# una-auxme/MeshGraphNets.jl

Measured on AMD Instinct MI355X. Metric: processor-step edges/s, higher is better.
Workload: dtype f32; 1 GPU; M-1M jittered-grid triangulation 1000x1000: N=1000000 nodes, E=5992002 directed edges, L=128, hidden_layers=2, 15 processor steps per bench step, fp32 storage, fp16x2 split MFMA (every fp32 operand = two fp16 pieces after a power-of-two scaling per weight chunk / per activation row, three exact piece products per fp32 product on v_mfma_f32_32x32x16_f16), fp32 accumulate; held to the fp32 tolerance; partition=single partition, edge_order=engine re-sorts by receiver once per trajectory (mgn_set_graph)

## Files before the change

### meshgraphnets.jl_amd/csrc/kernels.h

```cpp
#pragma once
#include <hip/hip_runtime.h>
#include <stdint.h>

namespace mgn {

constexpr int TILE = 32;
constexpr int MAX_CHUNKS = 9;

enum { T_B1 = 0, T_B2, T_B3, T_GAMMA, T_BETA, T_BQ, T_LN, T_COUNT };

struct GenMlp {
    const float* chunk[4];
    const float* tabs;
    int32_t nmid;
    int32_t use;
};

struct EdgeArgs {
    const int32_t* snd;
    const int32_t* rcv;
    int64_t E;
    int32_t ntiles;
    const float* P;
    const float* Q;
// ... 46 lines not shown
    float h2_s[9], h2_rs[9], h2_b2pos;
};

struct EncNodeArgs {
    int32_t n, ntiles;
    const int32_t* gid;
    const float* srcA; int32_t wa;
    const float* srcB; int32_t wb;
    const float* scale;
    const float* shift;
    const float* w1f;
    float* V; float* P; float* Q;
    const float* chunk[MAX_CHUNKS];
    const float* tabs;
    GenMlp gen;
    const uint16_t* splith[4];
    float h2_rs[4];
};

struct EncEdgeArgs {
    int64_t E; int32_t ntiles;
    const int64_t* gid;
    const float* ef; int32_t Fe;
    const float* scale; const float* shift;
    const float* w1f;
    float* Elat;
    const float* chunk[MAX_CHUNKS];
    const float* tabs;
    GenMlp gen;
    const uint16_t* splith[2];
    float h2_rs[2];
};

struct DecArgs {
    int32_t n, ntiles;
    const float* V;
    const float* w3f;
    const float* b3;
    int32_t O;
    const float* oscale; const float* oshift;
    const float* mask;
    const int32_t* gid;
    float* out;
    const float* chunk[MAX_CHUNKS];
    const float* tabs;
    GenMlp gen;
    const uint16_t* splith[2];
    float h2_rs[2];
};

struct BfEdgeArgs {
    const int32_t* snd; const int32_t* rcv; int64_t E; int32_t ntiles; int32_t tile0;
    const uint16_t* P; const uint16_t* Q;
    uint16_t* Elat; uint16_t* AGG;
    uint16_t* CARRY;
    const uint16_t* chunk[3];
    const float* tabs;
    unsigned long long* stamps;
};
struct BfNodeArgs {
    int32_t n, ntiles; const int32_t* rowptr;
    uint16_t* V; const uint16_t* AGG; const uint16_t* CARRY; uint16_t* P; uint16_t* Q;
    const uint16_t* chunk[7];
    const float* tabs;
    int64_t zero_row; int32_t tile0;
    const int32_t* rowptr2; const uint16_t* AGG2; const uint16_t* CARRY2; int64_t zero_row2;
};
hipError_t launch_edge_bf16(const BfEdgeArgs& a, hipStream_t s);
hipError_t launch_node_bf16(const BfNodeArgs& a, hipStream_t s);
hipError_t launch_project_bf16(const BfNodeArgs& a, hipStream_t s);
hipError_t launch_tile_f32_to_bf16(const float* src, uint16_t* dst, int64_t ntiles, hipStream_t s);
hipError_t launch_tile_bf16_to_f32(const uint16_t* src, float* dst, int64_t ntiles, hipStream_t s);
hipError_t launch_scatter_prows(const float* src, int src_stride , float* dst, int64_t row0, int64_t rows, int L, hipStream_t s);
hipError_t launch_scatter_prows16(const uint16_t* src, int src_stride , uint16_t* dst, int64_t row0, int64_t rows, hipStream_t s);
bool prows_blocked();
hipError_t launch_gather_rows16(const uint16_t* src, const int32_t* idx, uint16_t* dst, int64_t rows, int dst_stride , hipStream_t s);

struct LaunchCfg { int blocks; int threads; size_t lds; };
hipError_t launch_node_split_h(const NodeArgs& a, const LaunchCfg& lc, hipStream_t s);
hipError_t launch_project_split_h(const NodeArgs& a, const LaunchCfg& lc, hipStream_t s);
hipError_t launch_edge_ring_h(const EdgeArgs& a, const LaunchCfg& lc, hipStream_t s);
size_t edge_ring_h_lds();
int edge_ring_h_streamed();
hipError_t launch_edge_ring(const EdgeArgs& a, const LaunchCfg& lc, hipStream_t s);
hipError_t launch_node_split(const NodeArgs& a, const LaunchCfg& lc, hipStream_t s);
hipError_t launch_project_split(const NodeArgs& a, const LaunchCfg& lc, hipStream_t s);

struct LinComb {
    int n;
    float c[7];
    const float* k[7];
};
hipError_t launch_lincomb(float* out, const float* u, const LinComb& lc, float dt, int64_t n, hipStream_t s);
hipError_t launch_overwrite(float* x, const float* frame, const uint8_t* mask, int64_t N, int O, hipStream_t s);
int errnorm_partials();
hipError_t launch_errnorm(const float* u, const float* unew, const LinComb& lc, float dt, float atol, float rtol, int64_t n,
                          double* partial, hipStream_t s);

bool launch_is_small(int ntiles);
bool node_split_size(int ntiles);
bool launch_is_small_edge(int ntiles_e);
int coop16_enabled();
int set_c16_edge_tiles(int t);
bool ring_hs_default();
bool coop16_size(int ntiles_e, int ntiles_n, bool ring_hs = false);
int last_edge_kernel();
int last_node_kernel();
int set_fp32_split(int on);
int fp32_split_enabled();
int set_split_f16(int on);
int split_f16_enabled();
int set_c16_split(int on);
int c16_split_enabled();
int set_c16_row_tiles(int rt);
int set_kernel_path(int p);
int get_kernel_path();
hipError_t launch_edge_step(int L, const EdgeArgs& a, hipStream_t s);
hipError_t launch_node_step(int L, const NodeArgs& a, hipStream_t s);
hipError_t launch_project(int L, const NodeArgs& a, hipStream_t s);
hipError_t launch_node_project_fused(int L, const NodeArgs& a, hipStream_t s, bool* launched);
hipError_t launch_node_ring_hs(const NodeArgs& a, const LaunchCfg& lc, hipStream_t s);
int node_ring_hs_enabled();
hipError_t launch_enc_node(int L, const EncNodeArgs& a, hipStream_t s);
hipError_t launch_enc_edge(int L, const EncEdgeArgs& a, hipStream_t s);
hipError_t launch_decode(int L, const DecArgs& a, hipStream_t s);
hipError_t launch_gather_rows(const float* src, const int32_t* idx, float* dst, int64_t rows, int L, int dst_stride , hipStream_t s);
hipError_t launch_rows_to_tiles(const float* src, const int64_t* gid64, const int32_t* gid32, float* dst, int64_t rows, int L, hipStream_t s);
hipError_t launch_tiles_to_rows(const float* src, const int64_t* gid64, const int32_t* gid32, float* dst, int64_t rows, int L, hipStream_t s);
hipError_t launch_randn_rows(float* dst, const int64_t* gid64, const int32_t* gid32, int64_t rows, int L,
                             uint64_t seed, hipStream_t s);
int kernels_prow_block();
int split_prow_block();
int checksum_partials();
hipError_t launch_checksum(const float* src, int64_t n, double* partials, hipStream_t s);

}
```

### meshgraphnets.jl_amd/csrc/kernels.hip

```cpp
#include "frag.hpp"
#include "kernels.h"
#include "tile_common.hpp"
#include "split_common.hpp"

#include <cstdlib>
#include <mutex>
#include <unordered_map>

namespace mgn {


template <int NT>
DEVINL void gen_hidden(f32x16 (&acc)[NT], f32x16 (&y)[NT], const GenMlp& g, int lane, int h) {
    constexpr int L = 32 * NT;
    relu_frag<NT>(acc);
    for (int m = 0; m < g.nmid; ++m) {
        tab_frag<NT>(y, g.tabs + m * L, h);
        mfma_chunk<NT, false>(y, acc, g.chunk[m], lane);
        relu_frag<NT>(y);
#pragma unroll
        for (int t = 0; t < NT; ++t) acc[t] = y[t];
    }
}
template <int NT>
// ... 2513 lines not shown

static int g_last_edge_kernel = 0;
int last_edge_kernel() { return g_last_edge_kernel; }
#define SET_LAST_EDGE(A, CODE)                                                            \
    do {                                                                                  \
        if (2 * (int64_t)(A).ntiles * TILE >= (A).E) g_last_edge_kernel = (CODE);         \
    } while (0)

hipError_t launch_edge_step(int L, const EdgeArgs& a, hipStream_t s) {
    if (a.ntiles <= 0) return hipSuccess;
    if (a.gen.use && a.ElatSrc) return hipErrorInvalidValue;
    if (a.gen.use) SET_LAST_EDGE(a, 1);
    if (a.gen.use) DISPATCH_GEN(L, (k_edge_step<4, 0, true>), (k_edge_step<2, 0, true>), (k_edge_step<1, 0, true>), a, a.ntiles);
    const int nres = resident_chunks(L, 3);
    LaunchCfg lc = tile_launch(L, a.ntiles, nres);
    if (a.c16 && L == 128 && a.chunk_t[0]) {
        SET_LAST_EDGE(a, 2);
        const int nht = 2 * a.ntiles;
        int rt = g_c16_rt ? g_c16_rt : (nht + num_cus() - 1) / num_cus();
        const bool sp16 = g_fp32_split && (g_c16_split & 1) && a.split16[0];
        const int rt_max = (sp16 && !a.bf && !g_c16_rt) ? 6 : 3;
        rt = rt < 1 ? 1 : (rt > rt_max ? rt_max : rt);
        LaunchCfg c16{(nht + rt - 1) / rt, 256, (size_t)rt * 2 * 8 * 64 * 16 + (size_t)rt * 2 * 64 * 4};
        if (g_fp32_split && (g_c16_split & 1) && a.split16[0] && (rt >= 2 || (g_c16_split & 4))) {
            c16.lds = (size_t)rt * 2 * 12 * 64 * 16 + (size_t)rt * 2 * 64 * 4;
            const bool h2 = g_split_f16 && a.split16h[0] && rt <= 4;
            SET_LAST_EDGE(a, h2 ? 15 : 12);
#define C16E(RT_, BF_) (h2 ? launch_k(k_edge_coop16m<RT_, BF_, 2>, a, c16, s) : launch_k(k_edge_coop16m<RT_, BF_, 1>, a, c16, s))
            if (a.bf) {
                if (rt == 3) return C16E(3, true);
                if (rt == 2) return C16E(2, true);
                return C16E(1, true);
            }
            if (rt == 6) return C16E(6, false);
            if (rt == 5) return C16E(5, false);
            if (rt == 4) return C16E(4, false);
            if (rt == 3) return C16E(3, false);
            if (rt == 2) return C16E(2, false);
            return C16E(1, false);
#undef C16E
        }
        if (a.bf) {
            if (rt == 3) return launch_k(k_edge_coop16m<3, true>, a, c16, s);
            if (rt == 2) return launch_k(k_edge_coop16m<2, true>, a, c16, s);
            return launch_k(k_edge_coop16m<1, true>, a, c16, s);
        }
        if (rt == 3) return launch_k(k_edge_coop16m<3, false>, a, c16, s);
        if (rt == 2) return launch_k(k_edge_coop16m<2, false>, a, c16, s);
        return launch_k(k_edge_coop16m<1, false>, a, c16, s);
    }
    if (a.ElatSrc) return hipErrorInvalidValue;
    static const int coop_edge_ring_env = [] { const char* e = getenv("MGN_COOP_EDGE_TILES_PER_CU_RING"); return e ? atoi(e) : 0; }();
    const bool ring_ok = L == 128 && g_fp32_split == 1 && a.split[0] && g_path == 0;
    const int coop_edge_ring = coop_edge_ring_env > 0 ? coop_edge_ring_env : ((ring_ok && g_split_f16 && a.splith[0] && edge_ring_h_streamed()) ? 2 : 3);
    if (coop_ok(L, a.ntiles, a.chunk_t, true) && !(ring_ok && a.ntiles > coop_edge_ring * num_cus())) {
        SET_LAST_EDGE(a, 3);
        LaunchCfg c4{a.ntiles, 256, coop_lds()};
        return coop_fence(a.ntiles) ? launch_k(k_edge_coop<true>, a, c4, s) : launch_k(k_edge_coop<false>, a, c4, s);
    }
    if (L == 128) {
        if (small_launch(a.ntiles) && !(ring_ok && a.ntiles > coop_edge_ring * num_cus())) {
            SET_LAST_EDGE(a, 4);
            lc.lds = (size_t)T_COUNT * L * 4 + 64;
            return launch_k(k_edge_step<4, 0>, a, lc, s);
        }
        if (g_fp32_split && a.split[0] && g_path == 0) {
            LaunchCfg ls = lc;
            ls.lds = (size_t)3 * 32768 + (size_t)3 * 16384 + (size_t)T_COUNT * L * 4 + 64;
            static const int ring_waves = [] { const char* e = getenv("MGN_RING_WAVES"); return e ? atoi(e) : 0; }();
            bool four = a.ntiles <= 20 * num_cus();
            if (g_split_f16 && a.splith[0] && edge_ring_h_streamed()) {
                const int r4 = (a.ntiles + 4 * num_cus() - 1) / (4 * num_cus()), r8 = (a.ntiles + 8 * num_cus() - 1) / (8 * num_cus());
                four = 0.62 * r4 < (double)r8;
            }
            if (ring_waves == 4 || (ring_waves == 0 && four)) {
                ls.threads = 256;
                const int rounds = (a.ntiles + 4 * num_cus() - 1) / (4 * num_cus());
                int blocks = (a.ntiles + 4 * rounds - 1) / (4 * rounds);
                if (blocks > num_cus()) blocks = num_cus();
                ls.blocks = ((blocks + NUM_XCD - 1) / NUM_XCD) * NUM_XCD;
            }
            if (g_split_f16 && a.splith[0]) {
                ls.lds = edge_ring_h_lds();
                SET_LAST_EDGE(a, edge_ring_h_streamed() ? (ls.threads == 256 ? 17 : 16) : (ls.threads == 256 ? 14 : 13));
                return launch_edge_ring_h(a, ls, s);
            }
            SET_LAST_EDGE(a, ls.threads == 256 ? 8 : 7);
            return launch_edge_ring(a, ls, s);
        }
        SET_LAST_EDGE(a, 9);
        lc.lds += (size_t)MGN_EDGE_JR * 64 * 4 * 4;
        const int nw = lc.blocks * (lc.threads / 64);
        const int rem = a.ntiles % nw, rounds = a.ntiles / nw;
        if (g_tail_coop && g_path == 0 && a.chunk_t[0] && rounds >= MGN_SPREAD_ROUNDS && rem > 0 && rem * 10 < nw * 6) {
            EdgeArgs body = a, tail = a;
            body.ntiles = a.ntiles - rem;
            tail.tile0 = a.tile0 + body.ntiles;
            tail.ntiles = rem;
            const hipError_t e = launch_k(k_edge_step<4, 2>, body, lc, s);
            if (e != hipSuccess) return e;
            LaunchCfg c4{rem, 256, coop_lds()};
            return launch_k(k_edge_coop<false>, tail, c4, s);
        }
        return launch_k(k_edge_step<4, 2>, a, lc, s);
    }
    if (L == 64) return launch_k(k_edge_step<2, 3>, a, lc, s);
    if (L == 32) return launch_k(k_edge_step<1, 3>, a, lc, s);
    return hipErrorInvalidValue;
}
static int g_last_node_kernel = 0;
int last_node_kernel() { return g_last_node_kernel; }
hipError_t launch_node_step(int L, const NodeArgs& a, hipStream_t s) {
    if (a.ntiles <= 0) return hipSuccess;
    if (a.mode != 2) g_last_node_kernel = a.gen.use ? 1 : (a.c16 && L == 128 && a.chunk_t[0]) ? 2 : coop_ok(L, a.ntiles, a.chunk_t) ? 3 : 7;
    if (a.gen.use) {
        if (a.mode == 2) return launch_project(L, a, s);
        if (a.AGG2) {
            if (a.mode == 1) return hipErrorInvalidValue;
            DISPATCH_GEN(L, (k_node_step<4, 0, false, 2, true>), (k_node_step<2, 0, false, 2, true>), (k_node_step<1, 0, false, 2, true>), a, a.ntiles);
        }
        if (a.mode == 1) DISPATCH_GEN(L, (k_node_step<4, 0, true, 1, true>), (k_node_step<2, 0, true, 1, true>), (k_node_step<1, 0, true, 1, true>), a, a.ntiles);
        DISPATCH_GEN(L, (k_node_step<4, 0, false, 1, true>), (k_node_step<2, 0, false, 1, true>), (k_node_step<1, 0, false, 1, true>), a, a.ntiles);
    }
    if (a.c16 && L == 128 && a.chunk_t[0]) {
        LaunchCfg c16{2 * a.ntiles, 256, (size_t)4 * 8 * 64 * 16 + 2 * 64 * 4};
        if (g_fp32_split && (g_c16_split & 2) && a.split16[0] && (!a.AGG2 || a.split16[6])) {
            c16.lds = (size_t)4 * 12 * 64 * 16 + 2 * 64 * 4;
            if (a.mode != 2) g_last_node_kernel = 8;
            if (g_split_f16 && a.split16h[0] && (!a.AGG2 || a.split16h[6])) {
                if (a.bf) return a.AGG2 ? launch_k(k_node_coop16<2, true, 2>, a, c16, s) : launch_k(k_node_coop16<1, true, 2>, a, c16, s);
                return a.AGG2 ? launch_k(k_node_coop16<2, false, 2>, a, c16, s) : launch_k(k_node_coop16<1, false, 2>, a, c16, s);
            }
            if (a.bf) return a.AGG2 ? launch_k(k_node_coop16<2, true, 1>, a, c16, s) : launch_k(k_node_coop16<1, true, 1>, a, c16, s);
            return a.AGG2 ? launch_k(k_node_coop16<2, false, 1>, a, c16, s) : launch_k(k_node_coop16<1, false, 1>, a, c16, s);
        }
        if (a.bf) return a.AGG2 ? launch_k(k_node_coop16<2, true>, a, c16, s) : launch_k(k_node_coop16<1, true>, a, c16, s);
        return a.AGG2 ? launch_k(k_node_coop16<2, false>, a, c16, s) : launch_k(k_node_coop16<1, false>, a, c16, s);
    }
    const bool split_node = L == 128 && a.mode == 0 && a.split[0] && (!a.AGG2 || a.split[6]) && node_split_size(a.ntiles);
    if (g_node16_mid && g_fp32_split && (g_c16_split & 2) && g_path == 0 && L == 128 && !a.bf && !a.AGG2 && a.mode != 2 && a.split16[0] &&
        coop_ok(L, a.ntiles, a.chunk_t) && !split_node) {
        LaunchCfg c16{2 * a.ntiles, 256, (size_t)4 * 12 * 64 * 16 + 2 * 64 * 4};
        g_last_node_kernel = 9;
        if (g_split_f16 && a.split16h[0]) return launch_k(k_node_coop16<1, false, 2, 5>, a, c16, s);
        return launch_k(k_node_coop16<1, false, 1, 5>, a, c16, s);
    }
    if (coop_ok(L, a.ntiles, a.chunk_t) && !split_node) {
        LaunchCfg c4{a.ntiles, 256, coop_lds()};
        if (coop_fence(a.ntiles)) return a.AGG2 ? launch_k(k_node_coop<true, true>, a, c4, s) : launch_k(k_node_coop<false, true>, a, c4, s);
        return a.AGG2 ? launch_k(k_node_coop<true, false>, a, c4, s) : launch_k(k_node_coop<false, false>, a, c4, s);
    }
    if (a.mode == 2) return launch_project(L, a, s);
    const bool proj = a.mode == 1;
    if (split_node) {
        LaunchCfg ls = tile_launch(L, a.ntiles, 2);
        ls.lds = (size_t)4 * 16384 * 2 + (size_t)T_COUNT * L * 4 + 64;
        if (g_split_f16 && a.splith[0] && !a.AGG2) {
            g_last_node_kernel = 10;
            return launch_node_split_h(a, ls, s);
        }
        g_last_node_kernel = a.AGG2 ? 6 : 5;
        return launch_node_split(a, ls, s);
    }
    const int nres = resident_chunks(L, proj ? 6 : 4);
    const LaunchCfg lc = tile_launch(L, a.ntiles, nres);
    if (a.AGG2) {
        if (proj) return hipErrorInvalidValue;
// ... 196 lines not shown
```

### meshgraphnets.jl_amd/csrc/split.hip

```cpp
#include <cstdlib>

#include "kernels.h"
#include "tile_common.hpp"
#include "split_common.hpp"

namespace mgn {

#ifndef MGN_SP_CARRY
#define MGN_SP_CARRY 1
#endif
#ifndef MGN_SP_BUFFER
#define MGN_SP_BUFFER 1
#endif

template <int D> struct SpRing { u32x4 r2[D], r3[D]; };
template <bool G2, bool G3, bool RELU, int D, bool G1 = false, int OFF = 0, bool PRIMED = false, bool NEXT = false>
DEVINL void sp_layer_otf(f32x16 (&acc)[4], const f32x16 (&in)[4], const u32x4* p1, const u32x4* p2, const u32x4* p3, int lane,
                         SpRing<D>* carry = nullptr, const u32x4* nx2 = nullptr, const u32x4* nx3 = nullptr) {
    const u32x4* w1 = p1 + lane;
    const u32x4* w2 = p2 + lane;
    const u32x4* w3 = p3 + lane;
#if MGN_SP_BUFFER
    const N16Buf b1 = n16_buf(G1 ? p1 : nullptr), b2 = n16_buf(G2 ? p2 : nullptr), b3 = n16_buf(G3 ? p3 : nullptr);
    const unsigned voff = (unsigned)lane * 16u;
// ... 1061 lines not shown
        asm volatile("s_nop 1");
        RG_SCAN_LEVEL(acc, c1, "row_shr:1 row_mask:0xf bank_mask:0xf");
        RG_SCAN_LEVEL(acc, c2s, "row_shr:2 row_mask:0xf bank_mask:0xf");
        RG_SCAN_LEVEL(acc, c4, "row_shr:4 row_mask:0xf bank_mask:0xf");
#if MGN_RINGH_SCAN_SKIP
        if (__builtin_amdgcn_ballot_w64(c8) != 0)
#endif
        {
            RG_SCAN_LEVEL(acc, c8, "row_shr:8 row_mask:0xf bank_mask:0xf");
        }
        RG_SCAN_LEVEL(acc, cx, "row_bcast:15 row_mask:0xa bank_mask:0xf");
        PHASE_FENCE();
        EST(5);
        const bool tail = valid && ((c == 31) || (reff != rnext));
        const int r_first = __builtin_amdgcn_readfirstlane(reff);
        const bool sl = (start == 0) && (ix.r_before == r_first);
        const bool sr = (c == 31) && (ix.r_after == reff);
        const bool to_carry = sl || sr;
        f32x4* dst = to_carry ? prow_ptr(a.CARRY, (int64_t)2 * tile + (sl ? 0 : 1), L, h) : tile_ptr(a.AGG, r >> 5, L, 32 * h + (r & 31));
#if defined(MGN_WHATIF_H) && (MGN_WHATIF_H & 32)
        if (tail && a.E < 0) store_frag<NT>(dst, to_carry ? STRIDE_PROW : STRIDE_TILE, acc);
#else
        if (tail) store_frag_pol<NT, MGN_AGG_STORE>(dst, to_carry ? STRIDE_PROW : STRIDE_TILE, acc);
#endif
        EST(6);
        PHASE_FENCE();
#if defined(MGN_WHATIF_H) && (MGN_WHATIF_H & 64)
        zero_frag<NT>(acc);
#elif defined(MGN_WHATIF_H) && (MGN_WHATIF_H & 8)
        load_frag<NT>(acc, prow_ptr(a.Q, lane & 31, L, h), STRIDE_PROW);
#else
        load_frag<NT>(acc, prow_ptr(a.Q, ixn.r >= 0 ? ixn.r : 0, L, h), STRIDE_PROW);
#endif
#if MGN_RINGH_ESTORE_LAST
        PHASE_FENCE();
#if defined(MGN_WHATIF_H) && (MGN_WHATIF_H & 2)
        if (valid && a.E < 0) ring_store_e(etile, er);
#else
        if (valid) ring_store_e(etile, er);
#endif
#endif
        EST(7);
        ix = ixn;
        tw.tile += tw.stride;
    }
}

constexpr int HS_W = 4;
#ifndef MGN_HS_PREMUL
#define MGN_HS_PREMUL 0
#endif
#ifndef MGN_HS_REQ_STEP
#define MGN_HS_REQ_STEP 0
#endif
#ifndef MGN_HS_AHEAD
#define MGN_HS_AHEAD 4
#endif
template <int NCH>
struct RsT {
    static constexpr int W = HS_W;
    static constexpr int WPL = 32 / W;
    static constexpr int NW = NCH * WPL;
    static constexpr int NB = 3;
    static constexpr int BUF = 2 * W * 64;
    static constexpr int AHEAD = MGN_HS_AHEAD;
    static constexpr int SLOTS = AHEAD - 1;
    static_assert(NW % NB == 0 && NW % SLOTS == 0 && AHEAD >= 3, "static window -> buffer / slot mapping");
};
typedef RsT<3> Rs;
template <int LYR>
DEVINL RhFrag rs_first(const u32x4* ring) {
    constexpr int b = (Rs::WPL * LYR) % Rs::NB;
    RhFrag f;
    f.h = ring[b * Rs::BUF];
    f.l = ring[b * Rs::BUF + 64];
    return f;
}
template <int NCH>
struct RsSrcT {
    const u32x4* w[NCH];
};
typedef RsSrcT<3> RsSrc;
DEVINL const u32x4* rs_src(const u32x4* chunk, int w, int e) { return chunk + ((e >> 6) & 1) * 2048 + (w * Rs::W + (e >> 7)) * 64 + (e & 63); }
template <int LYR, int FIN, int RFS = 0, int NWV = 8, bool WRAP = false, int NCH = 3, bool PREMUL = false>
DEVINL void hs_layer_ring(f32x16 (&acc)[4], f32x16 (&in)[4], u32x4* ring, const RsSrcT<NCH>& src, RhFrag& nx, u32x4 (&pend)[Rs::SLOTS][Rs::BUF / (NWV * 64)], int lane,
                          int tid, float sx, float cfin = 0.f, const float* btab = nullptr, const f32x4* rf = nullptr, const N16Buf* rfb = nullptr, int rfs_rt = 0, float premul = 1.f) {
    constexpr int ROT = 2;
    constexpr int W = Rs::W, WPL = Rs::WPL, NW = RsT<NCH>::NW, BUF = Rs::BUF, NB = Rs::NB;
    constexpr int LPT = BUF / (NWV * 64);
    f32x4 side[2 * ROT];
    if constexpr (!WRAP && RFS > 0) {
#pragma unroll
        for (int m = 0; m < 2 * ROT; ++m) side[m] = rf[m * RFS];
    }
    auto bias = [&](int sn, int u) {
        f32x2 b = {0.f, 0.f};
        if constexpr (FIN == 2) b = *reinterpret_cast<const f32x2*>(btab + 8 * (4 * (sn >> 1) + 2 * (sn & 1) + (u >> 1)) + 2 * (u & 1));
        return b;
    };
    unsigned ph[4], pl[4];
#pragma unroll
    for (int u = 0; u < 4; ++u) {
        const f32x2 b = bias(0, u);
        h2_split_pair<FIN>(ph[u], pl[u], in[0][2 * u], in[0][2 * u + 1], sx, cfin, b[0], b[1]);
    }
    unsigned voff[LPT];
#pragma unroll
    for (int i = 0; i < LPT; ++i) {
        const int e = i * NWV * 64 + tid;
        voff[i] = (unsigned)((((e >> 6) & 1) * 2048 + (e >> 7) * 64 + (e & 63)) * 16);
        asm volatile("" : "+v"(voff[i]));
    }
    __builtin_amdgcn_sched_barrier(0);
#pragma unroll
    for (int s = 0; s < 8; ++s) {
        unsigned nh[4], nl[4];
#pragma unroll
        for (int t = 0; t < 4; ++t) {
            const int it = 4 * s + t;
            const int gw = WPL * LYR + it / W;
            const u32x4 a1 = nx.h, a2 = nx.l;
            if (it % W == MGN_HS_REQ_STEP) {
                const int g2 = (gw + Rs::AHEAD) % NW, l2 = g2 / WPL, w2 = g2 % WPL;
#pragma unroll
                for (int i = 0; i < LPT; ++i)
                    pend[gw % Rs::SLOTS][i] = *reinterpret_cast<const u32x4*>(reinterpret_cast<const char*>(src.w[l2] + w2 * W * 64) + voff[i]);
            }
            if constexpr (RFS != 0) {
                if ((t & 1) && s < 8 - ROT) {
                    f32x4 v;
                    if constexpr (WRAP && RFS < 0) v = rf[(int64_t)(2 * s + (t >> 1)) * rfs_rt];
                    else if constexpr (WRAP) v = n16_ld(*rfb, (unsigned)lane * 16u, (2 * s + (t >> 1)) * 1024);
                    else v = rf[(2 * (s + ROT) + (t >> 1)) * RFS];
#pragma unroll
                    for (int i = 0; i < 4; ++i) in[s >> 1][8 * (s & 1) + 4 * (t >> 1) + i] = v[i];
                }
            }
            if (it + 1 < 32) {
                const int gn = WPL * LYR + (it + 1) / W;
                nx.h = ring[(gn % NB) * BUF + (((it + 1) % W) * 2) * 64];
                nx.l = ring[(gn % NB) * BUF + (((it + 1) % W) * 2 + 1) * 64];
            } else if (LYR < NCH - 1) {
                nx = rs_first<LYR + 1>(ring);
            }
            if (it % W == W - 1) {
                const int b2 = (gw + 2) % NB;
#pragma unroll
                for (int i = 0; i < LPT; ++i) ring[b2 * BUF + i * NWV * 64 + tid - lane] = pend[(gw + 2 - Rs::AHEAD + NW) % Rs::SLOTS][i];
            }
            if (s < 7) {
                const int sn = s + 1;
                const f32x2 b = bias(sn, t);
                h2_split_pair<FIN>(nh[t], nl[t], in[sn >> 1][8 * (sn & 1) + 2 * t], in[sn >> 1][8 * (sn & 1) + 2 * t + 1], sx, cfin, b[0], b[1]);
            }
            if constexpr (PREMUL) {
                if (s == 0) {
#pragma unroll
                    for (int k = 0; k < 16; ++k) acc[t][k] *= premul;
                }
            }
            const sp_f16x8 bh = h2_op(ph), bl = h2_op(pl);
            acc[t] = __builtin_amdgcn_mfma_f32_32x32x16_f16(h2_wop(a2), bh, acc[t], 0, 0, 0);
            acc[t] = __builtin_amdgcn_mfma_f32_32x32x16_f16(h2_wop(a1), bl, acc[t], 0, 0, 0);
            acc[t] = __builtin_amdgcn_mfma_f32_32x32x16_f16(h2_wop(a1), bh, acc[t], 0, 0, 0);
            __builtin_amdgcn_sched_barrier(0);
            if (it % W == W - 1) ring_barrier();
        }
#pragma unroll
        for (int u = 0; u < 4; ++u) {
            ph[u] = nh[u];
            pl[u] = nl[u];
        }
    }
    if constexpr (RFS > 0 && !WRAP) {
        f32x16 r[4];
#pragma unroll
        for (int u = 0; u < 8; ++u)
#pragma unroll
            for (int j = 0; j < 8; ++j)
                r[u >> 1][8 * (u & 1) + j] = u < ROT ? side[2 * u + (j >> 2)][j & 3] : in[(u - ROT) >> 1][8 * ((u - ROT) & 1) + j];
#pragma unroll
        for (int t = 0; t < 4; ++t) in[t] = r[t];
    }
}
template <int NWV>
__global__ __launch_bounds__(NWV * 64, NWV / 4) void k_edge_ring_hs(const EdgeArgs a) {
    constexpr int NT = 4, L = 128;
    constexpr int BUF = Rs::BUF, LPT = BUF / (NWV * 64);
    extern __shared__ __attribute__((aligned(16))) float smem[];
    const int lane0 = threadIdx.x & 63;
    const int wave = __builtin_amdgcn_readfirstlane(threadIdx.x >> 6);
    const int tid = (int)threadIdx.x;
    u32x4* ringbase = reinterpret_cast<u32x4*>(smem);
    f32x4* park = reinterpret_cast<f32x4*>(ringbase + Rs::NB * BUF) + wave * 1024;
    float* tb = reinterpret_cast<float*>(ringbase + Rs::NB * BUF) + NWV * 4096;
    copy_to_lds(tb, a.tabs, T_COUNT * L);
    RsSrc src;
    u32x4 pend[Rs::SLOTS][LPT];
    {
        src.w[0] = reinterpret_cast<const u32x4*>(a.splith[2]);
        src.w[1] = reinterpret_cast<const u32x4*>(a.splith[0]);
        src.w[2] = reinterpret_cast<const u32x4*>(a.splith[1]);
#pragma unroll
        for (int w = 0; w < 2; ++w)
#pragma unroll
            for (int i = 0; i < LPT; ++i) ringbase[w * BUF + i * NWV * 64 + tid] = *rs_src(src.w[0], w, i * NWV * 64 + tid);
#pragma unroll
        for (int sl = 0; sl < Rs::SLOTS; ++sl)
#pragma unroll
            for (int i = 0; i < LPT; ++i) pend[sl][i] = *rs_src(src.w[0], 2, i * NWV * 64 + tid);
#pragma unroll
        for (int x = 2; x < Rs::AHEAD; ++x)
#pragma unroll
            for (int i = 0; i < LPT; ++i) pend[(x - Rs::AHEAD + Rs::NW) % Rs::SLOTS][i] = *rs_src(src.w[x / Rs::WPL], x % Rs::WPL, i * NWV * 64 + tid);
    }
    __syncthreads();
    const float sw1 = a.h2_s[2], rsw1 = a.h2_rs[2], rsw2 = a.h2_rs[0], rsw3 = a.h2_rs[1], b2pos = a.h2_b2pos;
    TileWalk tw0(a.ntiles, 0), tw(a.ntiles, wave);
    if (tw0.tile >= tw0.end) return;
    const int iters = (tw0.end - tw0.tile + tw0.stride - 1) / tw0.stride;
    if (MGN_RING_PHASES > 1 && iters >= 32) {
        const int ph = (int)(blockIdx.x / NUM_XCD) % MGN_RING_PHASES;
        for (int i = 0; i < ph * MGN_RINGH_PHASE_UNITS; ++i) __builtin_amdgcn_s_sleep(64);
    }
    const int last = a.tile0 + tw0.tile + (iters - 1) * tw0.stride;
    tw.tile += a.tile0;
    tw.end += a.tile0;
    auto clamp = [&](int t) { return t < tw.end ? t : last; };
    f32x16 acc[NT], y[NT];
    EdgeIdx ix = load_edge_idx_nb(a.snd, a.rcv, a.E, clamp(tw.tile), lane0 & 31);
    {
        const int h0 = lane0 >> 5;
        load_frag<NT>(acc, prow_ptr(a.Q, ix.r >= 0 ? ix.r : 0, L, h0), STRIDE_PROW);
        load_frag<NT>(y, tile_ptr(a.Elat, clamp(tw.tile), L, lane0), STRIDE_TILE);
    }
    int stamp_tile = 0;
    (void)stamp_tile;
    for (int j = 0; j < iters; ++j, ++stamp_tile) {
        OPAQUE_LANE();
        const bool on = tw.tile < tw.end;
        const int tile = clamp(tw.tile);
        const int nxt = clamp(tw.tile + tw.stride);
        const EdgeIdx ixn = load_edge_idx_nb(a.snd, a.rcv, a.E, nxt, c);
        const bool valid = on && ix.r >= 0;
        const int r = ix.r >= 0 ? ix.r : 0;
        f32x4* etile = tile_ptr(a.Elat, tile, L, lane);
        u32x4* ring = ringbase + lane;
        STAMP(0);
        __builtin_amdgcn_s_setprio(0);
        RhFrag nx = rs_first<0>(ring);
#pragma unroll
        for (int m = 0; m < 16; ++m) {
            f32x4 v;
#pragma unroll
            for (int i = 0; i < 4; ++i) v[i] = y[m >> 2][4 * (m & 3) + i];
            park[m * 64 + lane] = v;
        }
        const H2Scale x1 = h2_scale(h2_rowmax<true>(y));
        const int ps_row = ix.s;
#if MGN_HS_PREMUL
        hs_layer_ring<0, 0, STRIDE_PROW, NWV, false, 3, true>(acc, y, ring, src, nx, pend, lane, tid, x1.s, 0.f, nullptr, prow_ptr(a.P, ps_row, L, h), nullptr, 0, x1.s * sw1);
#else
        {
            const float cinv = x1.s * sw1;
#pragma unroll
            for (int t = 0; t < NT; ++t)
#pragma unroll
                for (int k = 0; k < 16; ++k) acc[t][k] *= cinv;
        }
        hs_layer_ring<0, 0, STRIDE_PROW, NWV>(acc, y, ring, src, nx, pend, lane, tid, x1.s, 0.f, nullptr, prow_ptr(a.P, ps_row, L, h));
#endif
        {
            const float c1 = x1.rs * rsw1;
#pragma unroll
            for (int t = 0; t < NT; ++t)
#pragma unroll
                for (int k = 0; k < 16; ++k) acc[t][k] = __builtin_fmaf(acc[t][k], c1, y[t][k]);
        }
        CST(1);
        const H2Scale x2 = h2_scale(h2_rowmax<false>(acc));
        zero_frag<NT>(y);
        CST(2);
        hs_layer_ring<1, 1, 0, NWV>(y, acc, ring, src, nx, pend, lane, tid, x2.s);
        CST(3);
        const float c2 = x2.rs * rsw2;
        const H2Scale x3 = h2_scale(__builtin_fmaf(h2_rowmax<false>(y), c2, b2pos));
        zero_frag<NT>(acc);
        CST(4);
        const N16Buf enb = n16_buf(a.Elat + (int64_t)nxt * (TILE * L), TILE * L * 4);
        hs_layer_ring<2, 2, STRIDE_TILE, NWV, true>(acc, y, ring, src, nx, pend, lane, tid, x3.s, c2, tb + T_B2 * L + 4 * h, nullptr, &enb);
        CST(5);
        EST(1);
        PHASE_FENCE();
        __builtin_amdgcn_s_setprio(MGN_PRIO);
#pragma unroll
        for (int m = 12; m < 16; ++m) {
            const f32x4 v = n16_ld(enb, (unsigned)lane * 16u, m * 1024);
#pragma unroll
            for (int i = 0; i < 4; ++i) y[3][4 * (m & 3) + i] = v[i];
        }
        {
            constexpr float invL = 1.0f / 128;
            const float c3 = x3.rs * rsw3;
            const f32x4* b34 = reinterpret_cast<const f32x4*>(tb + T_B3 * L) + h;
            float sm = 0.f;
#pragma unroll
            for (int t = 0; t < NT; ++t)
#pragma unroll
                for (int g = 0; g < 4; ++g) {
                    const f32x4 bv = b34[2 * (4 * t + g)];
#pragma unroll
                    for (int i = 0; i < 4; ++i) {
                        const float v = __builtin_fmaf(acc[t][4 * g + i], c3, bv[i]);
                        acc[t][4 * g + i] = v;
                        sm += v;
                    }
                }
            sm += __shfl_xor(sm, 32, 64);
            const float mean = sm * invL;
            float q = 0.f;
#pragma unroll
            for (int t = 0; t < NT; ++t)
#pragma unroll
                for (int k = 0; k < 16; ++k) {
                    const float d = acc[t][k] - mean;
                    acc[t][k] = d;
                    q += d * d;
                }
            q += __shfl_xor(q, 32, 64);
            const float rstd = ln_rstd_at(q * invL, tb + T_LN * L);
            const f32x4* g4 = reinterpret_cast<const f32x4*>(tb + T_GAMMA * L) + h;
            const f32x4* b4 = reinterpret_cast<const f32x4*>(tb + T_BETA * L) + h;
#pragma unroll
            for (int t = 0; t < NT; ++t) {
#pragma unroll
                for (int g = 0; g < 4; ++g) {
                    const f32x4 gv = g4[2 * (4 * t + g)];
                    const f32x4 bv = b4[2 * (4 * t + g)];
#pragma unroll
                    for (int i = 0; i < 4; ++i) acc[t][4 * g + i] = acc[t][4 * g + i] * rstd * gv[i] + bv[i];
                }
#pragma unroll
                for (int g = 0; g < 4; ++g) {
                    f32x4 v = park[(4 * t + g) * 64 + lane];
#pragma unroll
                    for (int i = 0; i < 4; ++i) v[i] += acc[t][4 * g + i];
                    if (valid) etile[(4 * t + g) * STRIDE_TILE] = v;
                }
            }
        }
        CST(6);
        EST(2);
        CST(7);
        EST(3);
        const int reff = ix.r >= 0 ? r : (-4 - c);
        const int rprev = __shfl_up(reff, 1, 32);
        const int rnext = __shfl_down(reff, 1, 32);
        const bool head = (c == 0) || (reff != rprev);
        const unsigned hm = (unsigned)__ballot(head);
        const int start = 31 - __clz((int)(hm & (0xFFFFFFFFu >> (31 - c))));
        const int st_in = max(start, c & 16);
        const bool c1 = (c - 1 >= st_in), c2s = (c - 2 >= st_in), c4 = (c - 4 >= st_in), c8 = (c - 8 >= st_in);
        const bool cx = (c >= 16) && (start <= 15);
        EST(4);
        PHASE_FENCE();
        asm volatile("s_nop 1");
        RG_SCAN_LEVEL(acc, c1, "row_shr:1 row_mask:0xf bank_mask:0xf");
        RG_SCAN_LEVEL(acc, c2s, "row_shr:2 row_mask:0xf bank_mask:0xf");
        RG_SCAN_LEVEL(acc, c4, "row_shr:4 row_mask:0xf bank_mask:0xf");
        if (__builtin_amdgcn_ballot_w64(c8) != 0)
        {
            RG_SCAN_LEVEL(acc, c8, "row_shr:8 row_mask:0xf bank_mask:0xf");
        }
        RG_SCAN_LEVEL(acc, cx, "row_bcast:15 row_mask:0xa bank_mask:0xf");
        PHASE_FENCE();
        EST(5);
        const bool tail = valid && ((c == 31) || (reff != rnext));
        const int r_first = __builtin_amdgcn_readfirstlane(reff);
        const bool sl = (start == 0) && (ix.r_before == r_first);
        const bool sr = (c == 31) && (ix.r_after == reff);
        const bool to_carry = sl || sr;
        f32x4* dst = to_carry ? prow_ptr(a.CARRY, (int64_t)2 * tile + (sl ? 0 : 1), L, h) : tile_ptr(a.AGG, r >> 5, L, 32 * h + (r & 31));
        if (tail) store_frag<NT>(dst, to_carry ? STRIDE_PROW : STRIDE_TILE, acc);
        EST(6);
        PHASE_FENCE();
        load_frag<NT>(acc, prow_ptr(a.Q, ixn.r >= 0 ? ixn.r : 0, L, h), STRIDE_PROW);
        EST(7);
        ix = ixn;
        tw.tile += tw.stride;
    }
}


#ifndef MGN_NODE_CPRIO_OLD
#define MGN_NODE_CPRIO_OLD 0
#endif
#ifndef MGN_NODE_CPRIO_YOUNG
#define MGN_NODE_CPRIO_YOUNG 0
#endif
#ifndef MGN_NODE_MPRIO
#define MGN_NODE_MPRIO MGN_PRIO
#endif
#define NODE_CHAIN_PRIO()                                                        \
    do {                                                                         \
        if (MGN_NODE_CPRIO_OLD == MGN_NODE_CPRIO_YOUNG) __builtin_amdgcn_s_setprio(MGN_NODE_CPRIO_OLD); \
        else if (wave < 4) __builtin_amdgcn_s_setprio(MGN_NODE_CPRIO_OLD);       \
        else __builtin_amdgcn_s_setprio(MGN_NODE_CPRIO_YOUNG);                   \
    } while (0)
#ifndef MGN_SP2_D3
#define MGN_SP2_D3 4
#endif
template <bool TWO>
__global__ __launch_bounds__(512, 2) void k_node_split(const NodeArgs a) {
    constexpr int NT = 4, L = 128, PC = 16384, D = MGN_SP2_D;
    extern __shared__ __attribute__((aligned(16))) float smem[];
    uint16_t* wl = reinterpret_cast<uint16_t*>(smem);
    {
        const bool fast = a.ntiles <= MGN_FAST_PRELOAD_TILES;
        copy_to_lds16(wl, a.split[2], PC, fast);
        copy_to_lds16(wl + PC, a.split[3], PC, fast);
        copy_to_lds16(wl + 2 * PC, a.split[0], PC, fast);
        copy_to_lds16(wl + 3 * PC, a.split[1], PC, fast);
    }
    float* tb = smem + 4 * PC / 2;
    copy_to_lds(tb, a.tabs, T_COUNT * L);
    __syncthreads();
    const u32x4* lvh = reinterpret_cast<const u32x4*>(wl);
    const u32x4* lah = reinterpret_cast<const u32x4*>(wl + PC);
    const u32x4* l2h = reinterpret_cast<const u32x4*>(wl + 2 * PC);
    const u32x4* l3h = reinterpret_cast<const u32x4*>(wl + 3 * PC);
    const u32x4* gv = reinterpret_cast<const u32x4*>(a.split[2]);
    const u32x4* ga = reinterpret_cast<const u32x4*>(a.split[3]);
    const u32x4* g2 = reinterpret_cast<const u32x4*>(a.split[0]);
    const u32x4* g3 = reinterpret_cast<const u32x4*>(a.split[1]);
    const int lane0 = threadIdx.x & 63;
    const int wave = __builtin_amdgcn_readfirstlane(threadIdx.x >> 6);
    stagger_second_half(wave, a.stagger);
    TileWalk tw(a.ntiles, wave, MGN_SPREAD_ROUNDS_NODE);
    if (tw.tile >= tw.end) return;
    f32x16 x[NT], acc[NT];
    load_frag<NT>(x, tile_ptr(a.V, tw.tile, L, lane0), STRIDE_TILE);
    for (;;) {
        OPAQUE_LANE();
        const int tile = tw.tile;
        const int next = tile + tw.stride;
        const bool has_next = next < tw.end;
        const int n = tile * TILE + c;
        const bool valid = n < a.n;
        const int nn = valid ? n : 0;
        f32x4* vtile = tile_ptr(a.V, tile, L, lane);
        NODE_CHAIN_PRIO();
        tab_frag<NT>(acc, tb + T_B1 * L, h);
#if defined(MGN_WHATIF_NODE) && (MGN_WHATIF_NODE & 1)
        sp_layer_otf<false, false, false, D>(acc, x, lvh, lvh, lvh, lane);
        LOAD_AGGREGATE(NT, x, a.rowptr, a.AGG, a.CARRY, a.zero_row);
        sp_layer_otf<false, false, false, D>(acc, x, lah, lah, lah, lane);
        tab_frag<NT>(x, tb + T_B2 * L, h);
        sp_layer_otf<false, false, true, D>(x, acc, l2h, l2h, l2h, lane);
        tab_frag<NT>(acc, tb + T_B3 * L, h);
        sp_layer_otf<false, false, true, D>(acc, x, l3h, l3h, l3h, lane);
#else
#if MGN_SP_CARRY
        constexpr int O1 = 32 % D, O2 = 64 % D, O3 = 96 % D;
        SpRing<D> rg;
        sp_layer_otf<true, true, false, D, false, 0, false, true>(acc, x, lvh, gv + 2048, gv + 4096, lane, &rg, ga + 2048, ga + 4096);
        LOAD_AGGREGATE(NT, x, a.rowptr, a.AGG, a.CARRY, a.zero_row);
        if constexpr (TWO) {
            sp_layer_otf<true, true, false, D, false, O1, true, false>(acc, x, lah, ga + 2048, ga + 4096, lane, &rg);
            const u32x4* gb = reinterpret_cast<const u32x4*>(a.split[6]);
            LOAD_AGGREGATE(NT, x, a.rowptr2, a.AGG2, a.CARRY2, a.zero_row2);
            sp_layer_otf<true, true, false, MGN_SP2_D3, true>(acc, x, gb, gb + 2048, gb + 4096, lane);
            tab_frag<NT>(x, tb + T_B2 * L, h);
// ... 454 lines not shown
#endif
        tw.tile += tw.stride;
    }
}

__global__ __launch_bounds__(512, 2) void k_project_split_h(const NodeArgs a) {
    constexpr int NT = 4, L = 128, PC = 16384;
    extern __shared__ __attribute__((aligned(16))) float smem[];
    uint16_t* wl = reinterpret_cast<uint16_t*>(smem);
    {
        const bool fast = a.ntiles <= MGN_FAST_PRELOAD_TILES;
        copy_to_lds16(wl, a.splith[4], 2 * PC, fast);
        copy_to_lds16(wl + 2 * PC, a.splith[5], 2 * PC, fast);
    }
    float* tb = smem + 4 * PC / 2;
    copy_to_lds(tb, a.tabs, T_COUNT * L);
    __syncthreads();
    const u32x4* lph = reinterpret_cast<const u32x4*>(wl);
    const u32x4* lpl = reinterpret_cast<const u32x4*>(wl + PC);
    const u32x4* lqh = reinterpret_cast<const u32x4*>(wl + 2 * PC);
    const u32x4* lql = reinterpret_cast<const u32x4*>(wl + 3 * PC);
    const float rswp = a.h2_rs[4], rswq = a.h2_rs[5];
    const int lane0 = threadIdx.x & 63;
    const int wave = __builtin_amdgcn_readfirstlane(threadIdx.x >> 6);
    TileWalk tw(a.ntiles, wave, MGN_SPREAD_ROUNDS_NODE);
    if (tw.tile >= tw.end) return;
    f32x16 x[NT], acc[NT];
    load_frag<NT>(x, tile_ptr(a.V, a.tile0 + tw.tile, L, lane0), STRIDE_TILE);
    for (;;) {
        OPAQUE_LANE();
        const int tile = a.tile0 + tw.tile;
        const int next = tw.tile + tw.stride;
        const bool has_next = next < tw.end;
        const int n = tile * TILE + c;
        const bool valid = n < a.n;
        const int nn = valid ? n : 0;
        NODE_CHAIN_PRIO();
        const H2Scale sv = h2_scale(h2_rowmax<true>(x));
        zero_frag<NT>(acc);
        h2_layer_otf<false, 0, 1>(acc, x, lph, lpl, lane, sv.s);
        __builtin_amdgcn_s_setprio(MGN_NODE_MPRIO);
        h2_scale_frag<NT>(acc, sv.rs * rswp);
        if (valid) store_frag_pol<NT, MGN_PROJ_STORE>(prow_ptr(a.P, nn, L, h), STRIDE_PROW, acc);
        NODE_CHAIN_PRIO();
        zero_frag<NT>(acc);
#if MGN_PROJ_VREFILL
        const f32x4* vnext = tile_ptr(a.V, a.tile0 + (has_next ? next : tw.tile), L, lane);
        h2_layer_otf<false, 0, 1, 0, false, false, MGN_PROJ_VREFILL, STRIDE_TILE>(acc, x, lqh, lql, lane, sv.s, 0.f, nullptr, nullptr, nullptr, vnext);
        __builtin_amdgcn_s_setprio(MGN_NODE_MPRIO);
        h2_load_tail<MGN_PROJ_VREFILL, STRIDE_TILE>(x, vnext);
        h2_finish_frag<NT>(acc, sv.rs * rswq, tb + T_BQ * L, h);
        if (valid) store_frag_pol<NT, MGN_PROJ_STORE>(prow_ptr(a.Q, nn, L, h), STRIDE_PROW, acc);
        if (!has_next) break;
#else
        h2_layer_otf<false, 0, 1>(acc, x, lqh, lql, lane, sv.s);
        __builtin_amdgcn_s_setprio(MGN_NODE_MPRIO);
        h2_finish_frag<NT>(acc, sv.rs * rswq, tb + T_BQ * L, h);
        if (valid) store_frag_pol<NT, MGN_PROJ_STORE>(prow_ptr(a.Q, nn, L, h), STRIDE_PROW, acc);
        if (!has_next) break;
        PHASE_FENCE();
        load_frag<NT>(x, tile_ptr(a.V, a.tile0 + next, L, lane), STRIDE_TILE);
#endif
        tw.tile = next;
    }
}

template <typename K, typename A>
static hipError_t sp_launch(K kern, const A& a, const LaunchCfg& lc, hipStream_t s, bool& attr_set) {
    if (!attr_set) {
        const hipError_t e = hipFuncSetAttribute(reinterpret_cast<const void*>(kern), hipFuncAttributeMaxDynamicSharedMemorySize, 160 * 1024);
        if (e != hipSuccess) return e;
        attr_set = true;
    }
    hipLaunchKernelGGL(kern, dim3(lc.blocks), dim3(lc.threads), lc.lds, s, a);
    return hipGetLastError();
}
hipError_t launch_edge_ring(const EdgeArgs& a, const LaunchCfg& lc, hipStream_t s) {
    static bool attr_set8 = false, attr_set4 = false;
    if (lc.threads == 256) return sp_launch(k_edge_ring<4>, a, lc, s, attr_set4);
    return sp_launch(k_edge_ring<8>, a, lc, s, attr_set8);
}
static int g_ringh_stream = [] { const char* e = getenv("MGN_RINGH_STREAM"); return e ? atoi(e) : 1; }();
int edge_ring_h_streamed() { return g_ringh_stream; }
hipError_t launch_edge_ring_h(const EdgeArgs& a, const LaunchCfg& lc, hipStream_t s) {
    static bool attr_set8 = false, attr_set4 = false, attr_s8 = false, attr_s4 = false;
    if (g_ringh_stream) {
        LaunchCfg ls = lc;
        ls.lds = (size_t)Rs::NB * Rs::BUF * 16 + (size_t)(lc.threads / 64) * 16384 + (size_t)T_COUNT * 128 * 4 + 64;
        if (lc.threads == 256) return sp_launch(k_edge_ring_hs<4>, a, ls, s, attr_s4);
        return sp_launch(k_edge_ring_hs<8>, a, ls, s, attr_s8);
    }
    if (lc.threads == 256) return sp_launch(k_edge_ring_h<4>, a, lc, s, attr_set4);
    return sp_launch(k_edge_ring_h<8>, a, lc, s, attr_set8);
}
size_t edge_ring_h_lds() { return (size_t)3 * 32768 + (size_t)Rh<MGN_RINGH_W>::NB * Rh<MGN_RINGH_W>::BUF * 16 + (size_t)T_COUNT * 128 * 4 + 64; }
hipError_t launch_node_split(const NodeArgs& a, const LaunchCfg& lc, hipStream_t s) {
    static bool attr_set = false;
    static bool attr_set2 = false;
    if (a.AGG2) return sp_launch(k_node_split<true>, a, lc, s, attr_set2);
    return sp_launch(k_node_split<false>, a, lc, s, attr_set);
}
hipError_t launch_node_split_h(const NodeArgs& a, const LaunchCfg& lc, hipStream_t s) {
    static bool attr_set = false;
    return sp_launch(k_node_split_h, a, lc, s, attr_set);
}
static int g_node_ring_hs = [] { const char* e = getenv("MGN_NODE_RING_HS"); return e ? atoi(e) : 1; }();
int node_ring_hs_enabled() { return g_node_ring_hs; }
hipError_t launch_node_ring_hs(const NodeArgs& a, const LaunchCfg& lc, hipStream_t s) {
    static bool attr_set = false;
    LaunchCfg ls = lc;
    ls.threads = 512;
    ls.lds = (size_t)Rs::NB * Rs::BUF * 16 + (size_t)8 * 16384 + (size_t)T_COUNT * 128 * 4 + 64;
    return sp_launch(k_node_ring_hs, a, ls, s, attr_set);
}
hipError_t launch_project_split_h(const NodeArgs& a, const LaunchCfg& lc, hipStream_t s) {
    static bool attr_set = false;
    return sp_launch(k_project_split_h, a, lc, s, attr_set);
}
hipError_t launch_project_split(const NodeArgs& a, const LaunchCfg& lc, hipStream_t s) {
    static bool attr_set = false;
    return sp_launch(k_project_split, a, lc, s, attr_set);
}

int split_prow_block() { return MGN_PROW_BLOCK; }

}
```

Before: 1.938 billion edges/s.

## Defer edge-latent write-back into next tile's MFMA layers and use policy stores

Adds an optional deferred mode to the streamed fp16-split edge ring kernel. Each updated edge-latent tile stays parked in LDS, and its global write-back is spread across the next tile's three MLP layers, so the stores overlap with MFMA work instead of clustering after layer norm. This mode is selected by an environment variable that defaults to off. Separately, the default 8-wave path now writes edge latents through a buffer store with a cache-policy hint instead of plain stores. The deferred path costs extra LDS traffic, more registers and more complex scheduling, and it needs a final drain after the loop.

```diff
diff --git a/meshgraphnets.jl_amd/csrc/kernels.h b/meshgraphnets.jl_amd/csrc/kernels.h
--- a/meshgraphnets.jl_amd/csrc/kernels.h
+++ b/meshgraphnets.jl_amd/csrc/kernels.h
@@ -152,6 +152,7 @@
 hipError_t launch_edge_ring_h(const EdgeArgs& a, const LaunchCfg& lc, hipStream_t s);
 size_t edge_ring_h_lds();
 int edge_ring_h_streamed();
+bool edge_ring_hs_deferred(int threads);
 hipError_t launch_edge_ring(const EdgeArgs& a, const LaunchCfg& lc, hipStream_t s);
 hipError_t launch_node_split(const NodeArgs& a, const LaunchCfg& lc, hipStream_t s);
 hipError_t launch_project_split(const NodeArgs& a, const LaunchCfg& lc, hipStream_t s);
diff --git a/meshgraphnets.jl_amd/csrc/kernels.hip b/meshgraphnets.jl_amd/csrc/kernels.hip
--- a/meshgraphnets.jl_amd/csrc/kernels.hip
+++ b/meshgraphnets.jl_amd/csrc/kernels.hip
@@ -2619,7 +2619,8 @@
             }
             if (g_split_f16 && a.splith[0]) {
                 ls.lds = edge_ring_h_lds();
-                SET_LAST_EDGE(a, edge_ring_h_streamed() ? (ls.threads == 256 ? 17 : 16) : (ls.threads == 256 ? 14 : 13));
+                const bool four_w = ls.threads == 256, defer = edge_ring_hs_deferred(ls.threads);
+                SET_LAST_EDGE(a, edge_ring_h_streamed() ? (four_w ? (defer ? 19 : 17) : (defer ? 18 : 16)) : (four_w ? 14 : 13));
                 return launch_edge_ring_h(a, ls, s);
             }
             SET_LAST_EDGE(a, ls.threads == 256 ? 8 : 7);
diff --git a/meshgraphnets.jl_amd/csrc/split.hip b/meshgraphnets.jl_amd/csrc/split.hip
--- a/meshgraphnets.jl_amd/csrc/split.hip
+++ b/meshgraphnets.jl_amd/csrc/split.hip
@@ -1167,9 +1167,42 @@
 };
 typedef RsSrcT<3> RsSrc;
 DEVINL const u32x4* rs_src(const u32x4* chunk, int w, int e) { return chunk + ((e >> 6) & 1) * 2048 + (w * Rs::W + (e >> 7)) * 64 + (e & 63); }
-template <int LYR, int FIN, int RFS = 0, int NWV = 8, bool WRAP = false, int NCH = 3, bool PREMUL = false>
+struct EDrain {
+    f32x4* park;
+    N16Buf b;
+    bool on;
+    f32x4 v[2];
+};
+#ifndef MGN_HS_DRAIN_POL
+#define MGN_HS_DRAIN_POL 2
+#endif
+#ifndef MGN_HS_DRAIN_W0
+#define MGN_HS_DRAIN_W0 0
+#endif
+template <int DR> constexpr int hd_step(int m) {
+    return DR == 1 ? 4 * (m >> 1) : DR == 3 ? (m < 8 ? 4 * (8 + 2 * m) : 4 * (m - 8)) : MGN_HS_DRAIN_W0 == 0 ? 4 * (m + (m >> 1)) : 4 * (MGN_HS_DRAIN_W0 + m);
+}
+template <int DR> constexpr bool hd_parks(int m) { return DR == 1 || (DR == 3 && m >= 8); }
+template <int DR>
+DEVINL void hd_read(EDrain& d, const f32x16 (&in)[4], int m) {
+    d.v[m & 1] = d.park[m * 64];
+    if (hd_parks<DR>(m)) {
+        f32x4 e;
+#pragma unroll
+        for (int i = 0; i < 4; ++i) e[i] = in[m >> 2][4 * (m & 3) + i];
+        d.park[m * 64] = e;
+    }
+}
+template <int LYR, int FIN, int RFS = 0, int NWV = 8, bool WRAP = false, int NCH = 3, bool PREMUL = false, int DR = 0>
 DEVINL void hs_layer_ring(f32x16 (&acc)[4], f32x16 (&in)[4], u32x4* ring, const RsSrcT<NCH>& src, RhFrag& nx, u32x4 (&pend)[Rs::SLOTS][Rs::BUF / (NWV * 64)], int lane,
-                          int tid, float sx, float cfin = 0.f, const float* btab = nullptr, const f32x4* rf = nullptr, const N16Buf* rfb = nullptr, int rfs_rt = 0, float premul = 1.f) {
+                          int tid, float sx, float cfin = 0.f, const float* btab = nullptr, const f32x4* rf = nullptr, const N16Buf* rfb = nullptr, int rfs_rt = 0, float premul = 1.f,
+                          EDrain* dr = nullptr) {
+    static_assert(DR == 0 || NCH == 3, "the drain schedule spans the three chains of an edge tile");
+    if constexpr (DR != 0 && LYR == 0) {
+#pragma unroll
+        for (int m = 0; m < 16; ++m)
+            if (hd_step<DR>(m) < 2) hd_read<DR>(*dr, in, m);
+    }
     constexpr int ROT = 2;
     constexpr int W = Rs::W, WPL = Rs::WPL, NW = RsT<NCH>::NW, BUF = Rs::BUF, NB = Rs::NB;
     constexpr int LPT = BUF / (NWV * 64);
@@ -1211,6 +1244,19 @@
                 for (int i = 0; i < LPT; ++i)
                     pend[gw % Rs::SLOTS][i] = *reinterpret_cast<const u32x4*>(reinterpret_cast<const char*>(src.w[l2] + w2 * W * 64) + voff[i]);
             }
+            if constexpr (DR != 0) {
+                const int q = 32 * LYR + it;
+#pragma unroll
+                for (int m = 0; m < 16; ++m)
+#if defined(MGN_WHATIF_HS) && (MGN_WHATIF_HS & 8)
+                    if (q == hd_step<DR>(m) && dr->on && rfs_rt < 0) n16_st_pol<MGN_HS_DRAIN_POL>(dr->b, (unsigned)lane * 16u, m * 1024, dr->v[m & 1]);
+#else
+                    if (q == hd_step<DR>(m) && dr->on) n16_st_pol<MGN_HS_DRAIN_POL>(dr->b, (unsigned)lane * 16u, m * 1024, dr->v[m & 1]);
+#endif
+#pragma unroll
+                for (int m = 0; m < 16; ++m)
+                    if (q == hd_step<DR>(m) - 2) hd_read<DR>(*dr, in, m);
+            }
             if constexpr (RFS != 0) {
                 if ((t & 1) && s < 8 - ROT) {
                     f32x4 v;
@@ -1268,9 +1314,16 @@
         for (int t = 0; t < 4; ++t) in[t] = r[t];
     }
 }
-template <int NWV>
+#ifndef MGN_HS_EST_POL
+#define MGN_HS_EST_POL 2
+#endif
+#ifndef MGN_HS_DEFER_LAYOUT
+#define MGN_HS_DEFER_LAYOUT 1
+#endif
+template <int NWV, bool DEFER = false>
 __global__ __launch_bounds__(NWV * 64, NWV / 4) void k_edge_ring_hs(const EdgeArgs a) {
     constexpr int NT = 4, L = 128;
+    constexpr int DR = DEFER ? MGN_HS_DEFER_LAYOUT : 0;
     constexpr int BUF = Rs::BUF, LPT = BUF / (NWV * 64);
     extern __shared__ __attribute__((aligned(16))) float smem[];
     const int lane0 = threadIdx.x & 63;
@@ -1319,6 +1372,9 @@
         load_frag<NT>(acc, prow_ptr(a.Q, ix.r >= 0 ? ix.r : 0, L, h0), STRIDE_PROW);
         load_frag<NT>(y, tile_ptr(a.Elat, clamp(tw.tile), L, lane0), STRIDE_TILE);
     }
+    EDrain dr;
+    dr.b = n16_buf(a.Elat, TILE * L * 4);
+    dr.on = false;
     int stamp_tile = 0;
     (void)stamp_tile;
     for (int j = 0; j < iters; ++j, ++stamp_tile) {
@@ -1329,17 +1385,24 @@
         const EdgeIdx ixn = load_edge_idx_nb(a.snd, a.rcv, a.E, nxt, c);
         const bool valid = on && ix.r >= 0;
         const int r = ix.r >= 0 ? ix.r : 0;
+#if defined(MGN_WHATIF_HS) && (MGN_WHATIF_HS & 4)
+        f32x4* etile = tile_ptr(a.Elat, a.tile0 + wave, L, lane);
+#else
         f32x4* etile = tile_ptr(a.Elat, tile, L, lane);
+#endif
         u32x4* ring = ringbase + lane;
         STAMP(0);
         __builtin_amdgcn_s_setprio(0);
         RhFrag nx = rs_first<0>(ring);
-#pragma unroll
-        for (int m = 0; m < 16; ++m) {
-            f32x4 v;
-#pragma unroll
-            for (int i = 0; i < 4; ++i) v[i] = y[m >> 2][4 * (m & 3) + i];
-            park[m * 64 + lane] = v;
+        dr.park = park + lane;
+        if constexpr (!DEFER) {
+#pragma unroll
+            for (int m = 0; m < 16; ++m) {
+                f32x4 v;
+#pragma unroll
+                for (int i = 0; i < 4; ++i) v[i] = y[m >> 2][4 * (m & 3) + i];
+                park[m * 64 + lane] = v;
+            }
         }
         const H2Scale x1 = h2_scale(h2_rowmax<true>(y));
         const int ps_row = ix.s;
@@ -1353,7 +1416,8 @@
 #pragma unroll
                 for (int k = 0; k < 16; ++k) acc[t][k] *= cinv;
         }
-        hs_layer_ring<0, 0, STRIDE_PROW, NWV>(acc, y, ring, src, nx, pend, lane, tid, x1.s, 0.f, nullptr, prow_ptr(a.P, ps_row, L, h));
+        hs_layer_ring<0, 0, STRIDE_PROW, NWV, false, 3, false, DR>(acc, y, ring, src, nx, pend, lane, tid, x1.s, 0.f, nullptr, prow_ptr(a.P, ps_row, L, h),
+                                                                   nullptr, 0, 1.f, &dr);
 #endif
         {
             const float c1 = x1.rs * rsw1;
@@ -1366,18 +1430,26 @@
         const H2Scale x2 = h2_scale(h2_rowmax<false>(acc));
         zero_frag<NT>(y);
         CST(2);
-        hs_layer_ring<1, 1, 0, NWV>(y, acc, ring, src, nx, pend, lane, tid, x2.s);
+        hs_layer_ring<1, 1, 0, NWV, false, 3, false, DR>(y, acc, ring, src, nx, pend, lane, tid, x2.s, 0.f, nullptr, nullptr, nullptr, 0, 1.f, &dr);
         CST(3);
         const float c2 = x2.rs * rsw2;
         const H2Scale x3 = h2_scale(__builtin_fmaf(h2_rowmax<false>(y), c2, b2pos));
         zero_frag<NT>(acc);
         CST(4);
         const N16Buf enb = n16_buf(a.Elat + (int64_t)nxt * (TILE * L), TILE * L * 4);
-        hs_layer_ring<2, 2, STRIDE_TILE, NWV, true>(acc, y, ring, src, nx, pend, lane, tid, x3.s, c2, tb + T_B2 * L + 4 * h, nullptr, &enb);
+        hs_layer_ring<2, 2, STRIDE_TILE, NWV, true, 3, false, DR>(acc, y, ring, src, nx, pend, lane, tid, x3.s, c2, tb + T_B2 * L + 4 * h, nullptr, &enb, 0, 1.f, &dr);
         CST(5);
         EST(1);
         PHASE_FENCE();
         __builtin_amdgcn_s_setprio(MGN_PRIO);
+        const N16Buf eb = n16_buf(a.Elat + (int64_t)tile * (TILE * L), TILE * L * 4);
+#if MGN_HS_DEFER_LAYOUT >= 2
+        f32x4 er[2][4];
+        if constexpr (DR >= 2) {
+#pragma unroll
+            for (int g = 0; g < 4; ++g) er[0][g] = n16_ld(eb, (unsigned)lane * 16u, g * 1024);
+        }
+#endif
 #pragma unroll
         for (int m = 12; m < 16; ++m) {
             const f32x4 v = n16_ld(enb, (unsigned)lane * 16u, m * 1024);
@@ -1425,12 +1497,35 @@
 #pragma unroll
                     for (int i = 0; i < 4; ++i) acc[t][4 * g + i] = acc[t][4 * g + i] * rstd * gv[i] + bv[i];
                 }
+#if MGN_HS_DEFER_LAYOUT >= 2
+                if constexpr (DR >= 2) {
+                    if (t + 1 < NT && !hd_parks<DR>(4 * (t + 1))) {
+#pragma unroll
+                        for (int g = 0; g < 4; ++g) er[(t + 1) & 1][g] = n16_ld(eb, (unsigned)lane * 16u, (4 * (t + 1) + g) * 1024);
+                    }
+                }
+#endif
 #pragma unroll
                 for (int g = 0; g < 4; ++g) {
-                    f32x4 v = park[(4 * t + g) * 64 + lane];
+                    const int m = 4 * t + g;
+                    f32x4 v;
+#if MGN_HS_DEFER_LAYOUT >= 2
+                    if (DR >= 2 && !hd_parks<DR>(m)) v = er[t & 1][g];
+                    else
+#endif
+                    v = park[m * 64 + lane];
 #pragma unroll
                     for (int i = 0; i < 4; ++i) v[i] += acc[t][4 * g + i];
-                    if (valid) etile[(4 * t + g) * STRIDE_TILE] = v;
+                    if constexpr (DEFER) park[m * 64 + lane] = v;
+#if defined(MGN_WHATIF_HS) && (MGN_WHATIF_HS & 1)
+                    else if (valid && a.E < 0) etile[m * STRIDE_TILE] = v;
+#elif defined(MGN_WHATIF_HS)
+                    else if (valid) etile[m * STRIDE_TILE] = v;
+#else
+                    else if constexpr (NWV == 8 && MGN_HS_EST_POL >= 0) {
+                        if (valid) n16_st_pol<MGN_HS_EST_POL>(eb, (unsigned)lane * 16u, m * 1024, v);
+                    } else if (valid) etile[m * STRIDE_TILE] = v;
+#endif
                 }
             }
         }
@@ -1466,13 +1561,27 @@
         const bool sr = (c == 31) && (ix.r_after == reff);
         const bool to_carry = sl || sr;
         f32x4* dst = to_carry ? prow_ptr(a.CARRY, (int64_t)2 * tile + (sl ? 0 : 1), L, h) : tile_ptr(a.AGG, r >> 5, L, 32 * h + (r & 31));
+#if defined(MGN_WHATIF_HS) && (MGN_WHATIF_HS & 2)
+        if (tail && a.E < 0) store_frag<NT>(dst, to_carry ? STRIDE_PROW : STRIDE_TILE, acc);
+#else
         if (tail) store_frag<NT>(dst, to_carry ? STRIDE_PROW : STRIDE_TILE, acc);
+#endif
         EST(6);
         PHASE_FENCE();
         load_frag<NT>(acc, prow_ptr(a.Q, ixn.r >= 0 ? ixn.r : 0, L, h), STRIDE_PROW);
         EST(7);
+        dr.b = eb;
+        dr.on = valid;
         ix = ixn;
         tw.tile += tw.stride;
+    }
+    if constexpr (DEFER) {
+        const int lane = lane0;
+#pragma unroll
+        for (int m = 0; m < 16; ++m) {
+            const f32x4 v = park[m * 64 + lane];
+            if (dr.on) n16_st(dr.b, (unsigned)lane * 16u, m * 1024, v);
+        }
     }
 }
 
@@ -2093,11 +2202,17 @@
 }
 static int g_ringh_stream = [] { const char* e = getenv("MGN_RINGH_STREAM"); return e ? atoi(e) : 1; }();
 int edge_ring_h_streamed() { return g_ringh_stream; }
+static int g_edge_defer = [] { const char* e = getenv("MGN_EDGE_DEFER"); return e ? atoi(e) : 0; }();
+bool edge_ring_hs_deferred(int threads) { return g_ringh_stream && (g_edge_defer == 2 || (g_edge_defer == 1 && threads != 256)); }
 hipError_t launch_edge_ring_h(const EdgeArgs& a, const LaunchCfg& lc, hipStream_t s) {
-    static bool attr_set8 = false, attr_set4 = false, attr_s8 = false, attr_s4 = false;
+    static bool attr_set8 = false, attr_set4 = false, attr_s8 = false, attr_s4 = false, attr_d8 = false, attr_d4 = false;
     if (g_ringh_stream) {
         LaunchCfg ls = lc;
         ls.lds = (size_t)Rs::NB * Rs::BUF * 16 + (size_t)(lc.threads / 64) * 16384 + (size_t)T_COUNT * 128 * 4 + 64;
+        if (edge_ring_hs_deferred(lc.threads)) {
+            if (lc.threads == 256) return sp_launch(k_edge_ring_hs<4, true>, a, ls, s, attr_d4);
+            return sp_launch(k_edge_ring_hs<8, true>, a, ls, s, attr_d8);
+        }
         if (lc.threads == 256) return sp_launch(k_edge_ring_hs<4>, a, ls, s, attr_s4);
         return sp_launch(k_edge_ring_hs<8>, a, ls, s, attr_s8);
     }
```

Result: faster. 1.961 billion edges/s, median of 6 (+1.2%).
